# si220/Forest-SLAM

Measured on AMD Instinct MI355X. Metric: stereo frames/sec (extract+match+local-BA) at 600p, 1/8 MI355X; ATE RMSE, higher is better.
Workload: dtype mixed: u8/u16 integer (FAST, BRIEF, Hamming, SGM), f32 (ORB angle/Harris, back-projection), f64 (PnP, BA incl. its Schur GEMM on f64 MFMA); 1 GPU; stereo VO front end, configs[1]: 960x600, ORB nfeatures=1000, BF-Hamming xcheck (L+R), SGBM-3way 96 disp, back-projection, PnP-RANSAC, local BA K=10; width=960, height=600, nfeatures=1000, local_ba=window K=10 per frame, 10 LM iterations (fvo_ba_windows), parallelism=seq-per-gpu x1

## Files before the change

### forest-slam_amd/csrc/fvo_internal.h

```cpp
#pragma once

#include <hip/hip_runtime.h>

#include <cstdint>
#include <string>
#include <vector>

#include "../../include/fvo.h"

#define FVO_MAX_LEVELS 12

struct OrbGeom {
  int nlevels;
  int w[FVO_MAX_LEVELS], h[FVO_MAX_LEVELS];
  float scale[FVO_MAX_LEVELS];
  int64_t off[FVO_MAX_LEVELS + 1];
  int row0[FVO_MAX_LEVELS + 1];
  int nfeat[FVO_MAX_LEVELS];
  int64_t cand_off[FVO_MAX_LEVELS + 1];
  int64_t total_px;
  int total_rows;
  int64_t cand_total;
  bool angle_pass;
};
// ... 2 lines not shown
  int32_t* xofs;
  int32_t* xc1;
  int32_t* yofs;
  int32_t* yc1;
  int64_t xoff[FVO_MAX_LEVELS], yoff[FVO_MAX_LEVELS];
};

constexpr int kBaMaxWindow = 21;
constexpr int kEmMaxCap = 5040;
constexpr int kRansacMaxIters = 1000;

#define FVO_KERNELS(X)                                                                                    \
  X(KN_ORB_COPY, "orb_copy_level0") X(KN_ORB_RESIZE, "orb_resize") X(KN_ORB_FAST, "orb_fast_score")       \
  X(KN_ORB_NMS_COUNT, "orb_nms_count") X(KN_ORB_ROW_SCAN, "orb_row_scan") X(KN_ORB_COMPACT, "orb_nms_compact") \
  X(KN_ORB_SELECT1, "orb_select_fast") X(KN_ORB_HARRIS, "orb_harris") X(KN_ORB_SELECT2, "orb_select_harris") \
  X(KN_ORB_OFFSETS, "orb_offsets") X(KN_ORB_ANGLE, "orb_angle") X(KN_ORB_BLUR, "orb_blur")                \
  X(KN_ORB_BRIEF, "orb_brief") X(KN_BF_ARGMIN, "bf_argmin") X(KN_BF_FINISH, "bf_finish")                  \
  X(KN_SG_VERT, "sgbm_vert") X(KN_SG_ROWS, "sgbm_rows") X(KN_SG_MEDIAN, "sgbm_median")                    \
  X(KN_BACKPROJECT, "backproject") X(KN_PNP, "pnp_ransac") X(KN_BA_STEREO, "ba_stereo")                   \
  X(KN_BA_BUILD, "ba_build") X(KN_BA_SOLVE, "ba_solve") X(KN_GATHER, "gather_matches")                    \
  X(KN_ESSENTIAL, "essential_ransac") X(KN_RECOVER, "recover_pose") X(KN_INGEST, "ingest_undistort_gray") \
  X(KN_MOTION_BLUR, "motion_blur") X(KN_MAP_XFORM, "map_transform") X(KN_VOXEL, "voxel_down_sample")      \
  X(KN_BF_KNN, "bf_knn") X(KN_BF_RATIO, "bf_ratio") X(KN_SPK_LOCAL, "speckle_local")                      \
  X(KN_SPK_SEAMS, "speckle_seams") X(KN_SPK_SUM, "speckle_sum") X(KN_SPK_APPLY, "speckle_apply")
#define FVO_KERNEL_ID(id, name) id,
enum FvoKernel { FVO_KERNELS(FVO_KERNEL_ID) KN_COUNT };
#undef FVO_KERNEL_ID

struct TimingRec {
  int id;
  hipEvent_t a, b;
};

struct fvo_ctx {
  int device = 0;
  uint64_t tmask = 0;
  std::vector<TimingRec> trecs;
  std::vector<hipEvent_t> tpool;
  fvo_config cfg{};
  OrbGeom g{};
  std::string err;
  int kp_cap = 0;
  int64_t ws_bytes = 0;
  std::vector<void*> allocs;
  uint8_t* pyr = nullptr;
  uint8_t* blur = nullptr;
  int orb_last_batch = 0;
  uint8_t* score = nullptr;
  uint32_t* cand = nullptr;
  uint64_t* hel = nullptr;
  int32_t* ncand = nullptr;
  int32_t* nsel1 = nullptr;
  int32_t* nsel2 = nullptr;
  int32_t* koff = nullptr;
  int32_t* scratch = nullptr;
  int64_t scratch_per = 0;
  ResizeTab rt{};
  int32_t* umax = nullptr;
  uint32_t* bf_rowkey = nullptr;
  uint32_t* bf_colkey = nullptr;
  uint32_t* bf_knn = nullptr;
  uint16_t* sg_V = nullptr;
  uint16_t* sg_M = nullptr;
  uint32_t* sg_ckpt = nullptr;
  int16_t* sg_raw = nullptr;
  uint64_t* sg_hand = nullptr;
  uint32_t* sg_ctl = nullptr;
  struct {
    bool valid = false;
    const void* matches = nullptr;
    const void* nmatch = nullptr;
    const void* stereo = nullptr;
    int nframes = 0, first_end = 0, nwin = 0, first_valid = 0;
  } ba_births;
  double* pnp_hyp = nullptr;
  int32_t* pnp_sub = nullptr;
  int16_t* rs_table = nullptr;
  int32_t rs_table_iters = 0;
  double* pnp_models = nullptr;
  double* pnp_ws = nullptr;
  int32_t* pnp_good = nullptr;
  void* pnp_state = nullptr;
  float* pnp_pts = nullptr;
  int32_t* pnp_plan = nullptr;
  int32_t pnp_max_iters = 0;
  uint8_t* fast_rec = nullptr;
  void* ba_ws = nullptr;
  int64_t ba_win_bytes = 0;
  hipStream_t ba_s2 = nullptr;
  hipEvent_t ba_fork = nullptr, ba_join = nullptr;
  double* em_x = nullptr;
  double* em_models = nullptr;
  int32_t* em_good = nullptr;
  int8_t* em_nmod = nullptr;
  double* em_ws = nullptr;
  void* em_state = nullptr;
  int32_t em_max_iters = 0;
  int32_t rectify_budget = FVO_RECTIFY_LDS_BYTES;
};

int fvo_fail(fvo_ctx* ctx, const std::string& msg);
#define FVO_HIP(ctx, expr)                                                                 \
  do {                                                                                     \
    hipError_t e_ = (expr);                                                                \
    if (e_ != hipSuccess) return fvo_fail(ctx, std::string(#expr) + ": " + hipGetErrorString(e_)); \
  } while (0)
#define FVO_LAUNCH_CHECK(ctx) FVO_HIP(ctx, hipGetLastError())

hipEvent_t fvo_event(fvo_ctx* ctx);
#define FVO_TIMED(ctx, id, s, ...)                               \
  do {                                                           \
    const bool t_ = ((ctx)->tmask >> (id)) & 1ull;               \
    hipEvent_t a_ = nullptr, b_ = nullptr;                       \
    if (t_) {                                                    \
      a_ = fvo_event(ctx);                                       \
      (void)hipEventRecord(a_, s);                               \
    }                                                            \
    __VA_ARGS__;                                                 \
    if (t_) {                                                    \
      b_ = fvo_event(ctx);                                       \
      (void)hipEventRecord(b_, s);                               \
      (ctx)->trecs.push_back(TimingRec{(int)(id), a_, b_});      \
    }                                                            \
  } while (0)

int orb_init(fvo_ctx* ctx);
int orb_run(fvo_ctx* ctx, const uint8_t* images, int batch, int64_t image_stride, int pitch, float* kp, uint8_t* desc,
            int32_t* counts, int cap, hipStream_t s);
int bf_init(fvo_ctx* ctx);
int bf_run(fvo_ctx* ctx, const uint8_t* q, const int32_t* nq, const uint8_t* t, const int32_t* nt, int batch, int cap,
           int32_t* matches, int32_t* nmatch, hipStream_t s);
int bf_knn_run(fvo_ctx* ctx, const uint8_t* q, const int32_t* nq, const uint8_t* t, const int32_t* nt, int batch,
               int cap, int k, int32_t* knn, hipStream_t s);
int bf_ratio_run(fvo_ctx* ctx, const uint8_t* q, const int32_t* nq, const uint8_t* t, const int32_t* nt, int batch,
                 int cap, double ratio, int mutual, int32_t* matches, int32_t* nmatch, hipStream_t s);
int sgbm_init(fvo_ctx* ctx);
int sgbm_run(fvo_ctx* ctx, const uint8_t* L, const uint8_t* R, int batch, int64_t image_stride, int pitch,
             int16_t* disp, int32_t* status, hipStream_t s);
int pose_init(fvo_ctx* ctx);
int ransac_table_init(fvo_ctx* ctx);
int orb_blur_debug(fvo_ctx* ctx);
int orb_score_debug(fvo_ctx* ctx);
int orb_retain_best_run(fvo_ctx* ctx, const float* keys, int n, int keep, int32_t* idx_out, int32_t* n_out,
                         hipStream_t s);
int backproject_run(fvo_ctx* ctx, const int16_t* disp, const float* kp0, const float* kp1, const int32_t* matches,
                    const int32_t* nmatch, int batch, int cap, const double* K, double baseline, float* P3, float* p2,
                    int32_t* npts, hipStream_t s);
int pnp_run(fvo_ctx* ctx, const float* P3, const float* p2, const int32_t* npts, int batch, int cap, const double* K,
            const double* dist, float reproj, double conf, int iters, double* rvec, double* tvec, double* T,
            int32_t* status, uint8_t* inliers, hipStream_t s);

int ingest_run(fvo_ctx* ctx, const uint8_t* bgr, int batch, int64_t sstride, int spitch, const double* K,
               const double* dist, uint8_t* gray, int64_t dstride, int dpitch, hipStream_t s);
int motion_blur_run(fvo_ctx* ctx, const uint8_t* img, int batch, int64_t sstride, int spitch, int ksize,
                    const int32_t* centers, const int32_t* ncent, int cap, uint8_t* mask, uint8_t* out,
                    int64_t dstride, int dpitch, hipStream_t s);
int map_transform_run(fvo_ctx* ctx, const float* pts, int stride, const int32_t* npts, int batch, int64_t cap,
                      const double* T, int32_t* count, int64_t map_cap, double* out64, float* out32, hipStream_t s);
int chain_poses_run(fvo_ctx* ctx, const double* T, const int32_t* status, const int32_t* npts, int n_seq, int n,
                    double* cum, double* cum_out, int32_t* npts_out, hipStream_t s);
struct FvoRegions {
  fvo_region r[FVO_MAX_REGIONS];
};
int copy_regions_run(fvo_ctx* ctx, int count, const fvo_region* regions, hipStream_t s);
int count_guard_run(fvo_ctx* ctx, const int32_t* cnt, const int32_t* q_cnt, int n, int sets, int32_t* status,
                    int32_t code, int32_t* nkp_out, hipStream_t s);
int64_t voxel_workspace_bytes(int64_t n);
// ... 60 lines not shown
```

### forest-slam_amd/csrc/pose.hip

```cpp
#include <cfloat>
#include <cstdlib>
#include <type_traits>

#include "fvo_device.h"
#include "ransac.h"

namespace {

constexpr int kChunk = 64;

constexpr int kBackprojectThreads = 256;

__global__ __launch_bounds__(kBackprojectThreads) void k_backproject(
    const int16_t* __restrict__ disp, const float* __restrict__ kp0, const float* __restrict__ kp1,
    const int32_t* __restrict__ matches, const int32_t* __restrict__ nmatch, int W, int H, int cap, StereoCamF K,
    float* __restrict__ P3, float* __restrict__ p2, int32_t* __restrict__ npts) {
  const int b = blockIdx.x;
  int n = nmatch[b];
  n = n < 0 ? 0 : (n > cap ? cap : n);
  __shared__ int s_w[16];
  __shared__ int s_carry;
  if (threadIdx.x == 0) s_carry = 0;
  __syncthreads();
  for (int base = 0; base < n; base += kBackprojectThreads) {
// ... 685 lines not shown
    double sum2 = 0.0;
    #pragma unroll
    for (int i = 0; i < NP; ++i) {
      const double* pw = &pws[3 * i];
      double Xc = dot3(&R[0], pw) + t[0], Yc = dot3(&R[3], pw) + t[1];
      double iz = 1.0 / (dot3(&R[6], pw) + t[2]);
      double ue = uc + fu * Xc * iz, ve = vc + fv * Yc * iz;
      double u = us[2 * i], v = us[2 * i + 1];
      sum2 += sqrt((u - ue) * (u - ue) + (v - ve) * (v - ve));
    }
    return sum2 / NP;
  }
  __device__ static void qr_solve(double* A, double* b, double* X) {
    const int nr = 6, nc = 4;
    double A1[4], A2[4];
    #pragma unroll
    for (int k = 0; k < nc; ++k) {
      double eta = fabs(A[k * nc + k]);
      #pragma unroll
      for (int i = k + 1; i < nr; ++i) eta = fmax(eta, fabs(A[i * nc + k]));
      if (eta == 0) return;
      double sum2 = 0.0, inv = 1. / eta;
      #pragma unroll
      for (int i = k; i < nr; ++i) {
        A[i * nc + k] *= inv;
        sum2 += A[i * nc + k] * A[i * nc + k];
      }
      double sigma = sqrt(sum2);
      if (A[k * nc + k] < 0) sigma = -sigma;
      A[k * nc + k] += sigma;
      A1[k] = sigma * A[k * nc + k];
      A2[k] = -eta * sigma;
      #pragma unroll
      for (int j = k + 1; j < nc; ++j) {
        double sum = 0;
        #pragma unroll
        for (int i = k; i < nr; ++i) sum += A[i * nc + k] * A[i * nc + j];
        double tau = sum / A1[k];
        #pragma unroll
        for (int i = k; i < nr; ++i) A[i * nc + j] -= tau * A[i * nc + k];
      }
    }
    #pragma unroll
    for (int j = 0; j < nc; ++j) {
      double tau = 0;
      #pragma unroll
      for (int i = j; i < nr; ++i) tau += A[i * nc + j] * b[i];
      tau /= A1[j];
      #pragma unroll
      for (int i = j; i < nr; ++i) b[i] -= tau * A[i * nc + j];
    }
    X[nc - 1] = b[nc - 1] / A2[nc - 1];
    #pragma unroll
    for (int i = nc - 2; i >= 0; --i) {
      double sum = 0;
      #pragma unroll
      for (int j = i + 1; j < nc; ++j) sum += A[i * nc + j] * X[j];
      X[i] = (b[i] - sum) / A2[i];
    }
  }
  __device__ static void gauss_newton(const double* L, const double* rho, double* betas) {
#pragma nounroll
    for (int it = 0; it < 5; ++it) {
      double A[24], b[6], x[4] = {0, 0, 0, 0};
      int o = 0;
      asm volatile("" : "+v"(o));
      #pragma unroll
      for (int i = 0; i < 6; ++i) {
        const double* r = L + o + 10 * i;
        A[i * 4 + 0] = 2 * r[0] * betas[0] + r[1] * betas[1] + r[3] * betas[2] + r[6] * betas[3];
        A[i * 4 + 1] = r[1] * betas[0] + 2 * r[2] * betas[1] + r[4] * betas[2] + r[7] * betas[3];
        A[i * 4 + 2] = r[3] * betas[0] + r[4] * betas[1] + 2 * r[5] * betas[2] + r[8] * betas[3];
        A[i * 4 + 3] = r[6] * betas[0] + r[7] * betas[1] + r[8] * betas[2] + 2 * r[9] * betas[3];
        b[i] = rho[o + i] - (r[0] * betas[0] * betas[0] + r[1] * betas[0] * betas[1] + r[2] * betas[1] * betas[1] +
                         r[3] * betas[0] * betas[2] + r[4] * betas[1] * betas[2] + r[5] * betas[2] * betas[2] +
                         r[6] * betas[0] * betas[3] + r[7] * betas[1] * betas[3] + r[8] * betas[2] * betas[3] +
                         r[9] * betas[3] * betas[3]);
      }
      qr_solve(A, b, x);
      #pragma unroll
      for (int i = 0; i < 4; ++i) betas[i] += x[i];
    }
  }
  template <int S>
  __device__ void build_mtm(double* __restrict__ MtM) {
    choose_control_points();
    barycentric();
#pragma unroll
    for (int i = 0; i < 144; ++i) MtM[i * S] = 0.0;
#pragma unroll
    for (int i = 0; i < NP; ++i) {
      const double* as = &alphas[4 * i];
      double u = us[2 * i], v = us[2 * i + 1];
      double M1[12], M2[12];
#pragma unroll
      for (int j = 0; j < 4; ++j) {
        M1[3 * j] = as[j] * fu; M1[3 * j + 1] = 0.0; M1[3 * j + 2] = as[j] * (uc - u);
        M2[3 * j] = 0.0; M2[3 * j + 1] = as[j] * fv; M2[3 * j + 2] = as[j] * (vc - v);
      }
#pragma unroll
      for (int a = 0; a < 12; ++a)
#pragma unroll
        for (int bb = 0; bb < 12; ++bb) MtM[(a * 12 + bb) * S] += M1[a] * M1[bb];
#pragma unroll
      for (int a = 0; a < 12; ++a)
#pragma unroll
        for (int bb = 0; bb < 12; ++bb) MtM[(a * 12 + bb) * S] += M2[a] * M2[bb];
    }
  }
  __device__ void prep(const double (*nv)[12], double* L, double* rho) const {
    const double* vv[4] = {nv[3], nv[2], nv[1], nv[0]};
    constexpr int pa[6] = {0, 0, 0, 1, 1, 2}, pb[6] = {1, 2, 3, 2, 3, 3};
#pragma unroll
    for (int i = 0; i < 6; ++i) {
      double dv[4][3];
#pragma unroll
      for (int a = 0; a < 4; ++a)
#pragma unroll
        for (int k = 0; k < 3; ++k) dv[a][k] = vv[a][3 * pa[i] + k] - vv[a][3 * pb[i] + k];
      double* r = L + 10 * i;
      r[0] = dot3(dv[0], dv[0]);
      r[1] = 2.0f * dot3(dv[0], dv[1]);
      r[2] = dot3(dv[1], dv[1]);
      r[3] = 2.0f * dot3(dv[0], dv[2]);
      r[4] = 2.0f * dot3(dv[1], dv[2]);
      r[5] = dot3(dv[2], dv[2]);
      r[6] = 2.0f * dot3(dv[0], dv[3]);
      r[7] = 2.0f * dot3(dv[1], dv[3]);
      r[8] = 2.0f * dot3(dv[2], dv[3]);
      r[9] = dot3(dv[3], dv[3]);
    }
    rho[0] = dist2(cws[0], cws[1]); rho[1] = dist2(cws[0], cws[2]); rho[2] = dist2(cws[0], cws[3]);
    rho[3] = dist2(cws[1], cws[2]); rho[4] = dist2(cws[1], cws[3]); rho[5] = dist2(cws[2], cws[3]);
  }
  __device__ double approx(int N, const double* L, const double* rho, const double (*nv)[12], double* R, double* t) {
    double betas[4];
    if (N == 1) {
      double A[24], b4[4];
      constexpr int c[4] = {0, 1, 3, 6};
#pragma unroll
      for (int i = 0; i < 6; ++i)
#pragma unroll
        for (int j = 0; j < 4; ++j) A[i * 4 + j] = L[i * 10 + c[j]];
      dsolve<6, 4>(A, rho, b4);
      double s = b4[0] < 0 ? -1.0 : 1.0;
      betas[0] = sqrt(s * b4[0]);
      betas[1] = s * b4[1] / betas[0];
      betas[2] = s * b4[2] / betas[0];
      betas[3] = s * b4[3] / betas[0];
    } else if (N == 2) {
      double A[18], b3[3];
#pragma unroll
      for (int i = 0; i < 6; ++i)
#pragma unroll
        for (int j = 0; j < 3; ++j) A[i * 3 + j] = L[i * 10 + j];
      dsolve<6, 3>(A, rho, b3);
      if (b3[0] < 0) {
        betas[0] = sqrt(-b3[0]);
        betas[1] = (b3[2] < 0) ? sqrt(-b3[2]) : 0.0;
      } else {
        betas[0] = sqrt(b3[0]);
        betas[1] = (b3[2] > 0) ? sqrt(b3[2]) : 0.0;
      }
      if (b3[1] < 0) betas[0] = -betas[0];
      betas[2] = 0.0;
      betas[3] = 0.0;
    } else {
      double A[30], b5[5];
#pragma unroll
      for (int i = 0; i < 6; ++i)
#pragma unroll
        for (int j = 0; j < 5; ++j) A[i * 5 + j] = L[i * 10 + j];
      dsolve<6, 5>(A, rho, b5);
      if (b5[0] < 0) {
        betas[0] = sqrt(-b5[0]);
        betas[1] = (b5[2] < 0) ? sqrt(-b5[2]) : 0.0;
      } else {
        betas[0] = sqrt(b5[0]);
        betas[1] = (b5[2] > 0) ? sqrt(b5[2]) : 0.0;
      }
      if (b5[1] < 0) betas[0] = -betas[0];
      betas[2] = b5[3] / betas[0];
      betas[3] = 0.0;
    }
    gauss_newton(L, rho, betas);
    return compute_R_and_t(nv, betas, R, t);
  }
};

using fvo_rs::RNG;
using fvo_rs::update_num_iters;

// ... 215 lines not shown
      for (int i = 0; i < 9; ++i) Rt[i] = -Rt[i];
#pragma unroll
    for (int i = 0; i < 3; ++i) T[i] = -(Rt[i * 3] * Mc[0] + Rt[i * 3 + 1] * Mc[1] + Rt[i * 3 + 2] * Mc[2]);
    if (lane == 0) {
#pragma unroll
      for (int i = 0; i < 9; ++i) sh.rt[i] = Rt[i];
#pragma unroll
      for (int i = 0; i < 3; ++i) sh.t3[i] = T[i];
    }
    for (int i = lane; i < n; i += 64) {
      const int j = i;
      double s0 = P3[3 * j], s1 = P3[3 * j + 1], s2 = P3[3 * j + 2];
      double X = Rt[0] * s0 + Rt[1] * s1 + Rt[2] * s2 + T[0];
      double Y = Rt[3] * s0 + Rt[4] * s1 + Rt[5] * s2 + T[1];
      double u = mn[2 * i], v = mn[2 * i + 1];
      double r0[9] = {X, Y, 1, 0, 0, 0, -u * X, -u * Y, -u};
      double r1[9] = {0, 0, 0, X, Y, 1, -v * X, -v * Y, -v};
      int k = 0;
#pragma unroll
      for (int a = 0; a < 9; ++a)
#pragma unroll
        for (int b = a; b < 9; ++b) LLp[k++] += r0[a] * r0[b] + r1[a] * r1[b];
    }
  }
#pragma unroll
  for (int k = 0; k < 78; ++k) {
    const double t = wave_sum(LLp[k]);
    if (lane == 0) sh.llp[k] = t;
  }
  __syncthreads();
  if (!planar) dlt12_null(sh.llp, sh.dlt[1], sh.dlt[2], sh.rrt);
  if (lane == 0) dlt_pose(sh, planar);
  __syncthreads();
  double prev[6];
  double lambdaLg10 = -3, prevErrNorm = DBL_MAX;
  int iters = 0;
  for (;;) {
    double e0 = lm_eval(sh, K, P3, p2, n, true);
#pragma unroll
    for (int i = 0; i < 6; ++i) prev[i] = sh.param[i];
    if (lane == 0) {
#pragma unroll
      for (int i = 0; i < 6; ++i) sh.prev[i] = prev[i];
    }
    __syncthreads();
    if (lane == 0) lm_step(sh, lambdaLg10);
    __syncthreads();
    if (iters == 0) prevErrNorm = e0;
    double errNorm;
    for (;;) {
      errNorm = lm_eval(sh, K, P3, p2, n, false);
      if (errNorm > prevErrNorm && ++lambdaLg10 <= 16) {
        if (lane == 0) lm_step(sh, lambdaLg10);
        __syncthreads();
        continue;
      }
      break;
    }
    lambdaLg10 = fmax(lambdaLg10 - 1, -16.0);
    double dn = 0, pn = 0;
#pragma unroll
    for (int i = 0; i < 6; ++i) {
      dn += (sh.param[i] - prev[i]) * (sh.param[i] - prev[i]);
      pn += prev[i] * prev[i];
    }
    double rel = sqrt(dn) / (sqrt(pn) + DBL_EPSILON);
    if (++iters >= 20 || rel < FLT_EPSILON) break;
    prevErrNorm = errNorm;
  }
  if (lane == 0) sh.flag = 1;
  __syncthreads();
}

struct PnpState {
  int maxGood, niters, best_it, n;
};

__global__ void k_pnp_table(int cap, int maxIters, int16_t* __restrict__ table) {
  const int n = blockIdx.x * blockDim.x + threadIdx.x;
  if (n < 6 || n > cap) return;
  fvo_rs::draw_subsets(n, maxIters, table + (int64_t)n * maxIters * 5);
}

__global__ void k_pnp_subsets(const int32_t* __restrict__ npts, int batch, int cap, int maxIters,
                              PnpState* __restrict__ state) {
  const int b = blockIdx.x * blockDim.x + threadIdx.x;
  if (b >= batch) return;
  int n = npts[b];
  n = n < 0 ? 0 : (n > cap ? cap : n);
  PnpState st;
  st.maxGood = 0;
  st.niters = maxIters;
  st.best_it = -1;
  st.n = n;
  state[b] = st;
}

constexpr int PNP_WS = 256;
constexpr int PW_NV = 0, PW_CWS = 48, PW_AL = 60, PW_PWS = 80, PW_US = 95, PW_MTM = 112;

constexpr int PNP_FIRST = 128;
constexpr int PNP_CS = 64, PNP_CA = 8, PNP_CB = 16;

__global__ __launch_bounds__(64) void k_pnp_plan(int batch, int maxIters, const PnpState* __restrict__ state,
                                                 int32_t* __restrict__ plan) {
  const int lane = threadIdx.x;
  int carry[3] = {0, 0, 0};
  const int C[3] = {PNP_CS, PNP_CA, PNP_CB};
  for (int b0 = 0; b0 < batch; b0 += 64) {
    const int b = b0 + lane;
    int rem = 0;
    if (b < batch) {
      const PnpState st = state[b];
      if (st.n >= 6) rem = max(0, min(st.niters, maxIters) - PNP_FIRST);
    }
#pragma unroll
    for (int k = 0; k < 3; ++k) {
      int v = (rem + C[k] - 1) / C[k];
#pragma unroll
      for (int o = 1; o < 64; o <<= 1) {
        const int y = __shfl_up(v, o, 64);
        if (lane >= o) v += y;
      }
      const int incl = v, excl = incl - (rem + C[k] - 1) / C[k];
      if (b < batch) plan[k * (batch + 1) + b] = carry[k] + excl;
      carry[k] += __shfl(incl, 63, 64);
    }
  }
  if (lane < 3) plan[lane * (batch + 1) + batch] = carry[lane];
}

__device__ __forceinline__ void pnp_unit(const int32_t* __restrict__ pre, int batch, int u, int C, int& b, int& base) {
  int lo = 0, hi = batch - 1;
  while (lo < hi) {
    const int mid = (lo + hi + 1) >> 1;
    if (pre[mid] <= u) lo = mid; else hi = mid - 1;
  }
  b = lo;
  base = PNP_FIRST + (u - pre[lo]) * C;
}

template <int C, typename Body>
__device__ __forceinline__ void pnp_units(const int32_t* __restrict__ plan, int k, int batch, int maxIters,
                                          const PnpState* __restrict__ state, Body body) {
  const int32_t* pre = plan ? plan + k * (batch + 1) : nullptr;
  const int total = plan ? pre[batch] : (int)blockIdx.x + 1;
  for (int u = blockIdx.x; u < total; u += gridDim.x) {
    int b, base, lim;
    if (plan) {
      pnp_unit(pre, batch, u, C, b, base);
      lim = maxIters;
    } else {
      b = blockIdx.y;
      base = u * C;
      lim = PNP_FIRST;
    }
    const PnpState st = state[b];
    const int hi = min(min(st.niters, maxIters), lim);
    if (st.n < 6 || base >= hi) continue;
    body(b, base, hi, st.n);
  }
}

__global__ __launch_bounds__(64, 4) void k_pnp_setup(const float* __restrict__ P3all, const float* __restrict__ p2all,
                                                  int cap, Cam K, int maxIters, int batch,
                                                  const int32_t* __restrict__ plan,
                                                  const int16_t* __restrict__ table, int table_iters,
                                                  const PnpState* __restrict__ state, double* __restrict__ ws) {
  extern __shared__ __attribute__((aligned(16))) double smt[];
  double* mt = smt + threadIdx.x;
  pnp_units<PNP_CS>(plan, 0, batch, maxIters, state, [&](int b, int base, int hi, int n) {
    const int it = base + threadIdx.x;
    if (it >= hi) return;
    const float* __restrict__ P3 = P3all + (int64_t)b * cap * 3;
    const float* __restrict__ p2 = p2all + (int64_t)b * cap * 2;
    double* w = ws + ((int64_t)b * maxIters + it) * PNP_WS;
    const int16_t* sb = table + ((int64_t)n * table_iters + it) * 5;
    EPnPd<5> e;
    e.fu = K.fx; e.fv = K.fy; e.uc = K.cx; e.vc = K.cy;
#pragma unroll
    for (int i = 0; i < 5; ++i) {
      int j = sb[i];
#pragma unroll
      for (int c = 0; c < 3; ++c) e.pws[3 * i + c] = (double)P3[j * 3 + c];
      double xy[2];
      dundistort(K, (double)p2[j * 2], (double)p2[j * 2 + 1], xy);
      float fx = (float)xy[0], fy = (float)xy[1];
      e.us[2 * i] = fx * K.fx + K.cx;
      e.us[2 * i + 1] = fy * K.fy + K.cy;
    }
    e.build_mtm<64>(mt);
#pragma unroll 8
    for (int k = 0; k < 144; ++k) w[PW_MTM + k] = mt[k * 64];
#pragma unroll
    for (int r = 0; r < 4; ++r)
#pragma unroll
      for (int k = 0; k < 3; ++k) w[PW_CWS + r * 3 + k] = e.cws[r][k];
#pragma unroll
    for (int k = 0; k < 20; ++k) w[PW_AL + k] = e.alphas[k];
#pragma unroll
    for (int k = 0; k < 15; ++k) w[PW_PWS + k] = e.pws[k];
#pragma unroll
    for (int k = 0; k < 10; ++k) w[PW_US + k] = e.us[k];
  });
}

__global__ __launch_bounds__(64) void k_pnp_hyp_a(int maxIters, int batch, const int32_t* __restrict__ plan,
                                                  const PnpState* __restrict__ state, double* __restrict__ ws) {
  __shared__ double su[8][144];
  const int g = threadIdx.x >> 3, l = threadIdx.x & 7;
  double* u = su[g];
  pnp_units<PNP_CA>(plan, 1, batch, maxIters, state, [&](int b, int base, int hi, int) {
    const int it = base + g;
    if (it >= hi) return;
    double* w = ws + ((int64_t)b * maxIters + it) * PNP_WS;
    for (int k = l; k < 144; k += 8) u[k] = w[PW_MTM + k];
    __builtin_amdgcn_s_waitcnt(0);
    __builtin_amdgcn_wave_barrier();
    jacobi12_null4_group(u, l, w + PW_NV);
  });
}

__global__ __launch_bounds__(64, 3) void k_pnp_hyp_b(const float* __restrict__ P3all, const float* __restrict__ p2all,
                                                  int cap, Cam K, float thr2, int maxIters, int batch,
                                                  const int32_t* __restrict__ plan,
                                                  const PnpState* __restrict__ state, const double* __restrict__ ws,
                                                  double* __restrict__ model, int32_t* __restrict__ good) {
  __shared__ double sL[16][66];
  const int g = threadIdx.x >> 2, l = threadIdx.x & 3;
  double* L = sL[g];
  pnp_units<PNP_CB>(plan, 2, batch, maxIters, state, [&](int b, int base, int hi, int n) {
    const int it = base + g;
    if (it >= hi) return;
    const float* __restrict__ P3 = P3all + (int64_t)b * cap * 3;
    const float* __restrict__ p2 = p2all + (int64_t)b * cap * 2;
    const double* w = ws + ((int64_t)b * maxIters + it) * PNP_WS;
    EPnPd<5, true> e;
    e.fu = K.fx; e.fv = K.fy; e.uc = K.cx; e.vc = K.cy;
    e.pws = w + PW_PWS;
    e.us = w + PW_US;
    e.alphas = w + PW_AL;
    e.cws = reinterpret_cast<const double (*)[3]>(w + PW_CWS);
    const double (*nv)[12] = reinterpret_cast<const double (*)[12]>(w + PW_NV);
    if (l == 0) e.prep(nv, L, L + 60);
    __builtin_amdgcn_s_waitcnt(0);
    __builtin_amdgcn_wave_barrier();
    double R[9], t[3];
    const double err = e.approx(l < 3 ? l + 1 : 3, L, L + 60, nv, R, t);
    const int gb = threadIdx.x & ~3;
    const double e1 = __shfl(err, gb + 1, 64), e2 = __shfl(err, gb + 2, 64);
    int sel = 0;
    double best = __shfl(err, gb, 64);
    if (e1 < best) { best = e1; sel = 1; }
    if (e2 < best) sel = 2;
#pragma unroll
    for (int k = 0; k < 9; ++k) R[k] = __shfl(R[k], gb + sel, 64);
#pragma unroll
    for (int k = 0; k < 3; ++k) t[k] = __shfl(t[k], gb + sel, 64);
    double r[3], dR[27];
    rod_R2r(R, r);
    if (l == 0) {
      double* mo = model + ((int64_t)b * maxIters + it) * 6;
      for (int i = 0; i < 3; ++i) { mo[i] = r[i]; mo[3 + i] = t[i]; }
    }
    rod_r2R(r, R, dR);
    int gcount = 0;
#pragma nounroll
    for (int i = l; i < n; i += 4) {
      double M[3] = {(double)P3[3 * i], (double)P3[3 * i + 1], (double)P3[3 * i + 2]}, uv[2];
      dproject(K, R, dR, t, M, uv, nullptr);
      float du = p2[2 * i] - (float)uv[0], dv = p2[2 * i + 1] - (float)uv[1];
      gcount += (du * du + dv * dv) <= thr2;
    }
    gcount += __shfl_xor(gcount, 1, 4);
    gcount += __shfl_xor(gcount, 2, 4);
    if (l == 0) good[(int64_t)b * maxIters + it] = gcount;
  });
}

__global__ __launch_bounds__(64) void k_pnp_replay(int maxIters, int it_lo, int it_hi, double conf,
                                                   const int32_t* __restrict__ good, PnpState* __restrict__ state) {
  const int b = blockIdx.x, lane = threadIdx.x;
  PnpState st = state[b];
  if (st.n < 6) return;
  for (int base = it_lo; base < it_hi && base < st.niters; base += 64) {
    const int it = base + lane;
    const int g = (it < it_hi && it < st.niters) ? good[(int64_t)b * maxIters + it] : 0;
    for (int j = 0; j < 64; ++j) {
      if (base + j >= it_hi || base + j >= st.niters) break;
      const int gj = __builtin_amdgcn_readlane(g, j);
      if (gj > max(st.maxGood, 4)) {
        st.best_it = base + j;
        st.maxGood = gj;
        st.niters = update_num_iters(conf, (double)(st.n - gj) / st.n, 5, st.niters);
      }
    }
  }
  if (lane == 0) state[b] = st;
}

__global__ __launch_bounds__(64, 2) void k_pnp_refine(const float* __restrict__ P3all, const float* __restrict__ p2all,
                                                   int cap, Cam K, float thr2, int maxIters,
                                                   const PnpState* __restrict__ state,
                                                   const double* __restrict__ model, double* __restrict__ rvec,
                                                   double* __restrict__ tvec, double* __restrict__ T,
                                                   int32_t* __restrict__ status, uint8_t* __restrict__ inliers,
                                                   int32_t* __restrict__ inl_idx, double* __restrict__ mn_buf,
                                                   float* __restrict__ pts) {
  __shared__ PnpShared sh;
  __shared__ float s_pts[5 * kRefineLds];
  const int b = blockIdx.x, lane = threadIdx.x;
  const PnpState st = state[b];
  const int n = st.n;
  const float* P3 = P3all + (int64_t)b * cap * 3;
  const float* p2 = p2all + (int64_t)b * cap * 2;
  double* Tout = T + (int64_t)b * 16;
  if (n < 6 || st.maxGood <= 0) {
    if (lane < 16) Tout[lane] = (lane % 5 == 0) ? 1.0 : 0.0;
    if (lane < 3) { rvec[b * 3 + lane] = 0; tvec[b * 3 + lane] = 0; }
    if (inliers)
      for (int i = lane; i < cap; i += 64) inliers[(int64_t)b * cap + i] = 0;
    if (lane == 0) status[b] = n < 6 ? -1 : 0;
    return;
  }
  const double* mo = model + ((int64_t)b * maxIters + st.best_it) * 6;
  if (lane < 6) sh.best[lane] = mo[lane];
  __syncthreads();
  int* inl = inl_idx + (int64_t)b * cap;
  {
    double r[3] = {sh.best[0], sh.best[1], sh.best[2]}, t[3] = {sh.best[3], sh.best[4], sh.best[5]};
    double R[9], dR[27];
    rod_r2R(r, R, dR);
    int carry = 0;
    for (int base = 0; base < n; base += 64) {
      int i = base + lane;
      bool f = false;
      if (i < n) {
        double M[3] = {(double)P3[3 * i], (double)P3[3 * i + 1], (double)P3[3 * i + 2]}, uv[2];
        dproject(K, R, dR, t, M, uv, nullptr);
        float du = p2[2 * i] - (float)uv[0], dv = p2[2 * i + 1] - (float)uv[1];
        f = du * du + dv * dv <= thr2;
        if (inliers) inliers[(int64_t)b * cap + i] = (uint8_t)f;
      }
      unsigned long long m = __ballot(f);
      if (f) {
        const int k = carry + __popcll(m & ((1ull << lane) - 1ull));
        inl[k] = i;
        if (k < kRefineLds) {
          s_pts[3 * k] = P3[3 * i];
          s_pts[3 * k + 1] = P3[3 * i + 1];
          s_pts[3 * k + 2] = P3[3 * i + 2];
          s_pts[3 * kRefineLds + 2 * k] = p2[2 * i];
          s_pts[3 * kRefineLds + 2 * k + 1] = p2[2 * i + 1];
        }
      }
      carry += __popcll(m);
    }
    if (inliers)
      for (int i = n + lane; i < cap; i += 64) inliers[(int64_t)b * cap + i] = 0;
    if (lane == 0) sh.ninl = carry;
  }
  __syncthreads();
  const int ninl = sh.ninl;
  const float* Pc = s_pts;
  const float* Qc = s_pts + 3 * kRefineLds;
  if (ninl > kRefineLds) {
    float* gP = pts + (int64_t)b * cap * 5;
    float* gQ = gP + 3 * cap;
    for (int k = lane; k < ninl; k += 64) {
      const int i = inl[k];
      gP[3 * k] = P3[3 * i];
      gP[3 * k + 1] = P3[3 * i + 1];
      gP[3 * k + 2] = P3[3 * i + 2];
      gQ[2 * k] = p2[2 * i];
      gQ[2 * k + 1] = p2[2 * i + 1];
    }
    __syncthreads();
    Pc = gP;
    Qc = gQ;
  }
  lm_refine(sh, K, Pc, Qc, ninl, mn_buf + (int64_t)b * cap * 2);
  double out[6];
  for (int i = 0; i < 6; ++i) out[i] = sh.flag ? sh.param[i] : sh.best[i];
  if (lane == 0) {
    double R[9];
    rod_r2R(out, R, nullptr);
    for (int i = 0; i < 3; ++i) {
      rvec[b * 3 + i] = out[i];
      tvec[b * 3 + i] = out[3 + i];
      Tout[i * 4 + 0] = R[i * 3];
      Tout[i * 4 + 1] = R[i * 3 + 1];
      Tout[i * 4 + 2] = R[i * 3 + 2];
      Tout[i * 4 + 3] = out[3 + i];
    }
    Tout[12] = 0; Tout[13] = 0; Tout[14] = 0; Tout[15] = 1;
    status[b] = 1;
  }
}

}

int pose_init(fvo_ctx* ctx) {
  ctx->pnp_max_iters = kRansacMaxIters;
  const int64_t B = ctx->cfg.max_batch, n = B * ctx->kp_cap, it = B * ctx->pnp_max_iters;
  int rc;
  if ((rc = fvo_alloc(ctx, &ctx->pnp_sub, n)) || (rc = fvo_alloc(ctx, &ctx->pnp_hyp, 2 * n)) ||
      (rc = ransac_table_init(ctx)) || (rc = fvo_alloc(ctx, &ctx->pnp_models, it * 6)) ||
      (rc = fvo_alloc(ctx, &ctx->pnp_ws, it * PNP_WS)) ||
      (rc = hipFuncSetAttribute((const void*)k_pnp_setup, hipFuncAttributeMaxDynamicSharedMemorySize,
                                144 * 64 * (int)sizeof(double)) == hipSuccess ? 0 : fvo_fail(ctx, "pnp: LDS attribute")) ||
      (rc = fvo_alloc(ctx, &ctx->pnp_good, it)) || (rc = fvo_alloc(ctx, (PnpState**)&ctx->pnp_state, B)) ||
      (rc = fvo_alloc(ctx, &ctx->pnp_plan, 3 * (B + 1))) || (rc = fvo_alloc(ctx, &ctx->pnp_pts, 5 * n)))
    return rc;
  return 0;
}

int ransac_table_init(fvo_ctx* ctx) {
  if (ctx->rs_table) return 0;
  ctx->rs_table_iters = kRansacMaxIters;
  int rc;
  if ((rc = fvo_alloc(ctx, &ctx->rs_table, (int64_t)(ctx->kp_cap + 1) * ctx->rs_table_iters * 5))) return rc;
  hipLaunchKernelGGL(k_pnp_table, dim3((ctx->kp_cap + 1 + 63) / 64), dim3(64), 0, 0, ctx->kp_cap,
                     ctx->rs_table_iters, ctx->rs_table);
  FVO_LAUNCH_CHECK(ctx);
  FVO_HIP(ctx, hipDeviceSynchronize());
  return 0;
}

int backproject_run(fvo_ctx* ctx, const int16_t* disp, const float* kp0, const float* kp1, const int32_t* matches,
                    const int32_t* nmatch, int batch, int cap, const double* K, double baseline, float* P3, float* p2,
                    int32_t* npts, hipStream_t s) {
  FVO_TIMED(ctx, KN_BACKPROJECT, s,
            hipLaunchKernelGGL(k_backproject, dim3(batch), dim3(kBackprojectThreads), 0, s, disp, kp0, kp1, matches,
                               nmatch, ctx->cfg.width, ctx->cfg.height, cap, stereo_cam(K, baseline), P3, p2, npts));
  FVO_LAUNCH_CHECK(ctx);
  return 0;
}

int pnp_run(fvo_ctx* ctx, const float* P3, const float* p2, const int32_t* npts, int batch, int cap, const double* K,
            const double* dist, float reproj, double conf, int iters, double* rvec, double* tvec, double* T,
            int32_t* status, uint8_t* inliers, hipStream_t s) {
  Cam c{K[0], K[4], K[2], K[5], {dist[0], dist[1], dist[2], dist[3], dist[4]}};
  const float thr2 = (float)((double)reproj * reproj);
  const int maxIters = iters;
  PnpState* st = (PnpState*)ctx->pnp_state;
  const int first = std::min(maxIters, PNP_FIRST);
  auto hyp = [&](const int32_t* plan, dim3 gs, dim3 ga, dim3 gb, int lo, int hi) {
    hipLaunchKernelGGL(k_pnp_setup, gs, dim3(64), 144 * 64 * sizeof(double), s, P3, p2, cap, c, maxIters, batch, plan,
                       ctx->rs_table, ctx->rs_table_iters, st, ctx->pnp_ws);
    hipLaunchKernelGGL(k_pnp_hyp_a, ga, dim3(64), 0, s, maxIters, batch, plan, st, ctx->pnp_ws);
    hipLaunchKernelGGL(k_pnp_hyp_b, gb, dim3(64), 0, s, P3, p2, cap, c, thr2, maxIters, batch, plan, st, ctx->pnp_ws,
                       ctx->pnp_models, ctx->pnp_good);
    hipLaunchKernelGGL(k_pnp_replay, dim3(batch), dim3(64), 0, s, maxIters, lo, hi, conf, ctx->pnp_good, st);
  };
  FVO_TIMED(ctx, KN_PNP, s, {
    hipLaunchKernelGGL(k_pnp_subsets, dim3((batch + 63) / 64), dim3(64), 0, s, npts, batch, cap, maxIters, st);
    hyp(nullptr, dim3((first + PNP_CS - 1) / PNP_CS, batch), dim3((first + PNP_CA - 1) / PNP_CA, batch),
        dim3((first + PNP_CB - 1) / PNP_CB, batch), 0, first);
    if (maxIters > first) {
      hipLaunchKernelGGL(k_pnp_plan, dim3(1), dim3(64), 0, s, batch, maxIters, st, ctx->pnp_plan);
      const int gs = batch * ((PNP_FIRST + PNP_CS - 1) / PNP_CS), ga = batch * ((PNP_FIRST + PNP_CA - 1) / PNP_CA),
                gb = batch * ((PNP_FIRST + PNP_CB - 1) / PNP_CB);
      hyp(ctx->pnp_plan, dim3(gs), dim3(ga), dim3(gb), first, maxIters);
    }
    hipLaunchKernelGGL(k_pnp_refine, dim3(batch), dim3(64), 0, s, P3, p2, cap, c, thr2, maxIters, st,
                       ctx->pnp_models, rvec, tvec, T, status, inliers, ctx->pnp_sub, ctx->pnp_hyp, ctx->pnp_pts);
  });
  FVO_LAUNCH_CHECK(ctx);
  return 0;
}
```

Before: 6000 frames/s.

## Fuse PnP setup into null-space kernel and fold plan, init and replay into neighbours

Measured after the change: 6033 frames/s, median of 6. No clear change (+0.6%).

```diff
diff --git a/forest-slam_amd/csrc/fvo_internal.h b/forest-slam_amd/csrc/fvo_internal.h
--- a/forest-slam_amd/csrc/fvo_internal.h
+++ b/forest-slam_amd/csrc/fvo_internal.h
@@ -108,7 +108,6 @@
   int32_t* pnp_good = nullptr;
   void* pnp_state = nullptr;
   float* pnp_pts = nullptr;
-  int32_t* pnp_plan = nullptr;
   int32_t pnp_max_iters = 0;
   uint8_t* fast_rec = nullptr;
   void* ba_ws = nullptr;
diff --git a/forest-slam_amd/csrc/pose.hip b/forest-slam_amd/csrc/pose.hip
--- a/forest-slam_amd/csrc/pose.hip
+++ b/forest-slam_amd/csrc/pose.hip
@@ -791,32 +791,6 @@
       for (int i = 0; i < 4; ++i) betas[i] += x[i];
     }
   }
-  template <int S>
-  __device__ void build_mtm(double* __restrict__ MtM) {
-    choose_control_points();
-    barycentric();
-#pragma unroll
-    for (int i = 0; i < 144; ++i) MtM[i * S] = 0.0;
-#pragma unroll
-    for (int i = 0; i < NP; ++i) {
-      const double* as = &alphas[4 * i];
-      double u = us[2 * i], v = us[2 * i + 1];
-      double M1[12], M2[12];
-#pragma unroll
-      for (int j = 0; j < 4; ++j) {
-        M1[3 * j] = as[j] * fu; M1[3 * j + 1] = 0.0; M1[3 * j + 2] = as[j] * (uc - u);
-        M2[3 * j] = 0.0; M2[3 * j + 1] = as[j] * fv; M2[3 * j + 2] = as[j] * (vc - v);
-      }
-#pragma unroll
-      for (int a = 0; a < 12; ++a)
-#pragma unroll
-        for (int bb = 0; bb < 12; ++bb) MtM[(a * 12 + bb) * S] += M1[a] * M1[bb];
-#pragma unroll
-      for (int a = 0; a < 12; ++a)
-#pragma unroll
-        for (int bb = 0; bb < 12; ++bb) MtM[(a * 12 + bb) * S] += M2[a] * M2[bb];
-    }
-  }
   __device__ void prep(const double (*nv)[12], double* L, double* rho) const {
     const double* vv[4] = {nv[3], nv[2], nv[1], nv[0]};
     constexpr int pa[6] = {0, 0, 0, 1, 1, 2}, pb[6] = {1, 2, 3, 2, 3, 3};
@@ -1198,139 +1172,144 @@
   fvo_rs::draw_subsets(n, maxIters, table + (int64_t)n * maxIters * 5);
 }
 
-__global__ void k_pnp_subsets(const int32_t* __restrict__ npts, int batch, int cap, int maxIters,
-                              PnpState* __restrict__ state) {
-  const int b = blockIdx.x * blockDim.x + threadIdx.x;
-  if (b >= batch) return;
-  int n = npts[b];
-  n = n < 0 ? 0 : (n > cap ? cap : n);
-  PnpState st;
-  st.maxGood = 0;
-  st.niters = maxIters;
-  st.best_it = -1;
-  st.n = n;
-  state[b] = st;
-}
-
-constexpr int PNP_WS = 256;
-constexpr int PW_NV = 0, PW_CWS = 48, PW_AL = 60, PW_PWS = 80, PW_US = 95, PW_MTM = 112;
+constexpr int PNP_WS = 112;
+constexpr int PW_NV = 0, PW_CWS = 48, PW_AL = 60, PW_PWS = 80, PW_US = 95;
 
 constexpr int PNP_FIRST = 128;
-constexpr int PNP_CS = 64, PNP_CA = 8, PNP_CB = 16;
-
-__global__ __launch_bounds__(64) void k_pnp_plan(int batch, int maxIters, const PnpState* __restrict__ state,
-                                                 int32_t* __restrict__ plan) {
+constexpr int PNP_CA = 8, PNP_CB = 16;
+
+__device__ __forceinline__ int pnp_clamp_n(int n, int cap) { return n < 0 ? 0 : (n > cap ? cap : n); }
+
+template <int C, typename Body>
+__device__ __forceinline__ void pnp_units(int batch, int cap, int maxIters,
+                                          const int32_t* __restrict__ npts, const PnpState* __restrict__ state,
+                                          Body body) {
+  __shared__ int pre[4][64];
   const int lane = threadIdx.x;
-  int carry[3] = {0, 0, 0};
-  const int C[3] = {PNP_CS, PNP_CA, PNP_CB};
-  for (int b0 = 0; b0 < batch; b0 += 64) {
-    const int b = b0 + lane;
-    int rem = 0;
-    if (b < batch) {
-      const PnpState st = state[b];
-      if (st.n >= 6) rem = max(0, min(st.niters, maxIters) - PNP_FIRST);
-    }
-#pragma unroll
-    for (int k = 0; k < 3; ++k) {
-      int v = (rem + C[k] - 1) / C[k];
+  const bool round2 = npts == nullptr;
+  int u = blockIdx.x, tot = 0;
+  for (int b0 = 0; b0 < (round2 ? batch : 1); b0 += 64) {
+    if (!round2) {
+      tot = u + 1;
+    } else {
+      const int bl = b0 + lane;
+      int n = 0, nit = 0, v = 0;
+      if (bl < batch) {
+        const PnpState st = state[bl];
+        n = st.n;
+        nit = min(st.niters, maxIters);
+        if (n >= 6) v = (max(0, nit - PNP_FIRST) + C - 1) / C;
+      }
+      int incl = v;
 #pragma unroll
       for (int o = 1; o < 64; o <<= 1) {
-        const int y = __shfl_up(v, o, 64);
-        if (lane >= o) v += y;
-      }
-      const int incl = v, excl = incl - (rem + C[k] - 1) / C[k];
-      if (b < batch) plan[k * (batch + 1) + b] = carry[k] + excl;
-      carry[k] += __shfl(incl, 63, 64);
-    }
-  }
-  if (lane < 3) plan[lane * (batch + 1) + batch] = carry[lane];
-}
-
-__device__ __forceinline__ void pnp_unit(const int32_t* __restrict__ pre, int batch, int u, int C, int& b, int& base) {
-  int lo = 0, hi = batch - 1;
-  while (lo < hi) {
-    const int mid = (lo + hi + 1) >> 1;
-    if (pre[mid] <= u) lo = mid; else hi = mid - 1;
-  }
-  b = lo;
-  base = PNP_FIRST + (u - pre[lo]) * C;
-}
-
-template <int C, typename Body>
-__device__ __forceinline__ void pnp_units(const int32_t* __restrict__ plan, int k, int batch, int maxIters,
-                                          const PnpState* __restrict__ state, Body body) {
-  const int32_t* pre = plan ? plan + k * (batch + 1) : nullptr;
-  const int total = plan ? pre[batch] : (int)blockIdx.x + 1;
-  for (int u = blockIdx.x; u < total; u += gridDim.x) {
-    int b, base, lim;
-    if (plan) {
-      pnp_unit(pre, batch, u, C, b, base);
-      lim = maxIters;
-    } else {
-      b = blockIdx.y;
-      base = u * C;
-      lim = PNP_FIRST;
-    }
-    const PnpState st = state[b];
-    const int hi = min(min(st.niters, maxIters), lim);
-    if (st.n < 6 || base >= hi) continue;
-    body(b, base, hi, st.n);
-  }
-}
-
-__global__ __launch_bounds__(64, 4) void k_pnp_setup(const float* __restrict__ P3all, const float* __restrict__ p2all,
-                                                  int cap, Cam K, int maxIters, int batch,
-                                                  const int32_t* __restrict__ plan,
-                                                  const int16_t* __restrict__ table, int table_iters,
-                                                  const PnpState* __restrict__ state, double* __restrict__ ws) {
-  extern __shared__ __attribute__((aligned(16))) double smt[];
-  double* mt = smt + threadIdx.x;
-  pnp_units<PNP_CS>(plan, 0, batch, maxIters, state, [&](int b, int base, int hi, int n) {
-    const int it = base + threadIdx.x;
+        const int y = __shfl_up(incl, o, 64);
+        if (lane >= o) incl += y;
+      }
+      incl += tot;
+      __builtin_amdgcn_wave_barrier();
+      pre[0][lane] = incl - v;
+      pre[1][lane] = incl;
+      pre[2][lane] = nit;
+      pre[3][lane] = n;
+      __builtin_amdgcn_s_waitcnt(0);
+      __builtin_amdgcn_wave_barrier();
+      tot = __shfl(incl, 63, 64);
+    }
+    while (u < tot) {
+      int b, base, hi, nn;
+      if (round2) {
+        const int src = __ffsll((unsigned long long)__ballot(pre[0][lane] <= u && u < pre[1][lane])) - 1;
+        b = b0 + src;
+        base = PNP_FIRST + (u - pre[0][src]) * C;
+        hi = pre[2][src];
+        nn = pre[3][src];
+      } else {
+        b = blockIdx.y;
+        base = u * C;
+        hi = min(maxIters, PNP_FIRST);
+        nn = pnp_clamp_n(npts[b], cap);
+      }
+      b = __builtin_amdgcn_readfirstlane(b);
+      base = __builtin_amdgcn_readfirstlane(base);
+      hi = __builtin_amdgcn_readfirstlane(hi);
+      nn = __builtin_amdgcn_readfirstlane(nn);
+      if (nn >= 6 && base < hi) body(b, base, hi, nn);
+      u += gridDim.x;
+    }
+  }
+}
+
+__global__ __launch_bounds__(64, 4) void k_pnp_null(const float* __restrict__ P3all, const float* __restrict__ p2all,
+                                                 const int32_t* __restrict__ npts, int cap, Cam K, int maxIters,
+                                                 int batch, const int16_t* __restrict__ table,
+                                                 int table_iters, const PnpState* __restrict__ state,
+                                                 double* __restrict__ ws) {
+  __shared__ double su[8][144];
+  __shared__ double sa[8][32];
+  const int g = threadIdx.x >> 3, l = threadIdx.x & 7;
+  double* u = su[g];
+  double* al = sa[g];
+  pnp_units<PNP_CA>(batch, cap, maxIters, npts, state, [&](int b, int base, int hi, int n) {
+    const int it = base + g;
     if (it >= hi) return;
     const float* __restrict__ P3 = P3all + (int64_t)b * cap * 3;
     const float* __restrict__ p2 = p2all + (int64_t)b * cap * 2;
     double* w = ws + ((int64_t)b * maxIters + it) * PNP_WS;
     const int16_t* sb = table + ((int64_t)n * table_iters + it) * 5;
-    EPnPd<5> e;
-    e.fu = K.fx; e.fv = K.fy; e.uc = K.cx; e.vc = K.cy;
-#pragma unroll
-    for (int i = 0; i < 5; ++i) {
-      int j = sb[i];
-#pragma unroll
-      for (int c = 0; c < 3; ++c) e.pws[3 * i + c] = (double)P3[j * 3 + c];
-      double xy[2];
-      dundistort(K, (double)p2[j * 2], (double)p2[j * 2 + 1], xy);
-      float fx = (float)xy[0], fy = (float)xy[1];
-      e.us[2 * i] = fx * K.fx + K.cx;
-      e.us[2 * i + 1] = fy * K.fy + K.cy;
-    }
-    e.build_mtm<64>(mt);
-#pragma unroll 8
-    for (int k = 0; k < 144; ++k) w[PW_MTM + k] = mt[k * 64];
-#pragma unroll
-    for (int r = 0; r < 4; ++r)
-#pragma unroll
-      for (int k = 0; k < 3; ++k) w[PW_CWS + r * 3 + k] = e.cws[r][k];
-#pragma unroll
-    for (int k = 0; k < 20; ++k) w[PW_AL + k] = e.alphas[k];
-#pragma unroll
-    for (int k = 0; k < 15; ++k) w[PW_PWS + k] = e.pws[k];
-#pragma unroll
-    for (int k = 0; k < 10; ++k) w[PW_US + k] = e.us[k];
-  });
-}
-
-__global__ __launch_bounds__(64) void k_pnp_hyp_a(int maxIters, int batch, const int32_t* __restrict__ plan,
-                                                  const PnpState* __restrict__ state, double* __restrict__ ws) {
-  __shared__ double su[8][144];
-  const int g = threadIdx.x >> 3, l = threadIdx.x & 7;
-  double* u = su[g];
-  pnp_units<PNP_CA>(plan, 1, batch, maxIters, state, [&](int b, int base, int hi, int) {
-    const int it = base + g;
-    if (it >= hi) return;
-    double* w = ws + ((int64_t)b * maxIters + it) * PNP_WS;
-    for (int k = l; k < 144; k += 8) u[k] = w[PW_MTM + k];
+    {
+      EPnPd<5> e;
+      e.fu = K.fx; e.fv = K.fy; e.uc = K.cx; e.vc = K.cy;
+#pragma unroll
+      for (int i = 0; i < 5; ++i) {
+        int j = sb[i];
+#pragma unroll
+        for (int c = 0; c < 3; ++c) e.pws[3 * i + c] = (double)P3[j * 3 + c];
+        double xy[2];
+        dundistort(K, (double)p2[j * 2], (double)p2[j * 2 + 1], xy);
+        float fx = (float)xy[0], fy = (float)xy[1];
+        e.us[2 * i] = fx * K.fx + K.cx;
+        e.us[2 * i + 1] = fy * K.fy + K.cy;
+      }
+      e.choose_control_points();
+      e.barycentric();
+      if (l == 0) {
+#pragma unroll
+        for (int k = 0; k < 20; ++k) al[k] = e.alphas[k];
+#pragma unroll
+        for (int k = 0; k < 10; ++k) al[20 + k] = e.us[k];
+#pragma unroll
+        for (int r = 0; r < 4; ++r)
+#pragma unroll
+          for (int k = 0; k < 3; ++k) w[PW_CWS + r * 3 + k] = e.cws[r][k];
+#pragma unroll
+        for (int k = 0; k < 20; ++k) w[PW_AL + k] = e.alphas[k];
+#pragma unroll
+        for (int k = 0; k < 15; ++k) w[PW_PWS + k] = e.pws[k];
+#pragma unroll
+        for (int k = 0; k < 10; ++k) w[PW_US + k] = e.us[k];
+      }
+    }
+    __builtin_amdgcn_s_waitcnt(0);
+    __builtin_amdgcn_wave_barrier();
+#pragma nounroll
+    for (int k = l; k < 144; k += 8) {
+      const int a = k / 12, bb = k - a * 12;
+      const int ja = a / 3, ca = a - ja * 3, jb = bb / 3, cb = bb - jb * 3;
+      double m = 0.0;
+#pragma unroll
+      for (int i = 0; i < 5; ++i) {
+        const double asa = al[4 * i + ja], asb = al[4 * i + jb];
+        const double pu = al[20 + 2 * i], pv = al[20 + 2 * i + 1];
+        const double m1a = ca == 0 ? asa * K.fx : (ca == 1 ? 0.0 : asa * (K.cx - pu));
+        const double m1b = cb == 0 ? asb * K.fx : (cb == 1 ? 0.0 : asb * (K.cx - pu));
+        const double m2a = ca == 0 ? 0.0 : (ca == 1 ? asa * K.fy : asa * (K.cy - pv));
+        const double m2b = cb == 0 ? 0.0 : (cb == 1 ? asb * K.fy : asb * (K.cy - pv));
+        m += m1a * m1b;
+        m += m2a * m2b;
+      }
+      u[k] = m;
+    }
     __builtin_amdgcn_s_waitcnt(0);
     __builtin_amdgcn_wave_barrier();
     jacobi12_null4_group(u, l, w + PW_NV);
@@ -1338,14 +1317,14 @@
 }
 
 __global__ __launch_bounds__(64, 3) void k_pnp_hyp_b(const float* __restrict__ P3all, const float* __restrict__ p2all,
-                                                  int cap, Cam K, float thr2, int maxIters, int batch,
-                                                  const int32_t* __restrict__ plan,
+                                                  const int32_t* __restrict__ npts, int cap, Cam K, float thr2,
+                                                  int maxIters, int batch,
                                                   const PnpState* __restrict__ state, const double* __restrict__ ws,
                                                   double* __restrict__ model, int32_t* __restrict__ good) {
   __shared__ double sL[16][66];
   const int g = threadIdx.x >> 2, l = threadIdx.x & 3;
   double* L = sL[g];
-  pnp_units<PNP_CB>(plan, 2, batch, maxIters, state, [&](int b, int base, int hi, int n) {
+  pnp_units<PNP_CB>(batch, cap, maxIters, npts, state, [&](int b, int base, int hi, int n) {
     const int it = base + g;
     if (it >= hi) return;
     const float* __restrict__ P3 = P3all + (int64_t)b * cap * 3;
@@ -1394,11 +1373,8 @@
   });
 }
 
-__global__ __launch_bounds__(64) void k_pnp_replay(int maxIters, int it_lo, int it_hi, double conf,
-                                                   const int32_t* __restrict__ good, PnpState* __restrict__ state) {
-  const int b = blockIdx.x, lane = threadIdx.x;
-  PnpState st = state[b];
-  if (st.n < 6) return;
+__device__ __forceinline__ void pnp_replay(PnpState& st, int b, int lane, int maxIters, int it_lo, int it_hi,
+                                           double conf, const int32_t* __restrict__ good) {
   for (int base = it_lo; base < it_hi && base < st.niters; base += 64) {
     const int it = base + lane;
     const int g = (it < it_hi && it < st.niters) ? good[(int64_t)b * maxIters + it] : 0;
@@ -1412,12 +1388,25 @@
       }
     }
   }
+}
+
+__global__ __launch_bounds__(64) void k_pnp_replay(const int32_t* __restrict__ npts, int cap, int maxIters, int it_hi,
+                                                   double conf, const int32_t* __restrict__ good,
+                                                   PnpState* __restrict__ state) {
+  const int b = blockIdx.x, lane = threadIdx.x;
+  PnpState st;
+  st.maxGood = 0;
+  st.niters = maxIters;
+  st.best_it = -1;
+  st.n = pnp_clamp_n(npts[b], cap);
+  if (st.n >= 6) pnp_replay(st, b, lane, maxIters, 0, it_hi, conf, good);
   if (lane == 0) state[b] = st;
 }
 
 __global__ __launch_bounds__(64, 2) void k_pnp_refine(const float* __restrict__ P3all, const float* __restrict__ p2all,
-                                                   int cap, Cam K, float thr2, int maxIters,
-                                                   const PnpState* __restrict__ state,
+                                                   int cap, Cam K, float thr2, int maxIters, double conf,
+                                                   PnpState* __restrict__ state,
+                                                   const int32_t* __restrict__ good,
                                                    const double* __restrict__ model, double* __restrict__ rvec,
                                                    double* __restrict__ tvec, double* __restrict__ T,
                                                    int32_t* __restrict__ status, uint8_t* __restrict__ inliers,
@@ -1426,8 +1415,12 @@
   __shared__ PnpShared sh;
   __shared__ float s_pts[5 * kRefineLds];
   const int b = blockIdx.x, lane = threadIdx.x;
-  const PnpState st = state[b];
+  PnpState st = state[b];
   const int n = st.n;
+  if (n >= 6 && maxIters > PNP_FIRST) {
+    pnp_replay(st, b, lane, maxIters, PNP_FIRST, maxIters, conf, good);
+    if (lane == 0) state[b] = st;
+  }
   const float* P3 = P3all + (int64_t)b * cap * 3;
   const float* p2 = p2all + (int64_t)b * cap * 2;
   double* Tout = T + (int64_t)b * 16;
@@ -1523,10 +1516,8 @@
   if ((rc = fvo_alloc(ctx, &ctx->pnp_sub, n)) || (rc = fvo_alloc(ctx, &ctx->pnp_hyp, 2 * n)) ||
       (rc = ransac_table_init(ctx)) || (rc = fvo_alloc(ctx, &ctx->pnp_models, it * 6)) ||
       (rc = fvo_alloc(ctx, &ctx->pnp_ws, it * PNP_WS)) ||
-      (rc = hipFuncSetAttribute((const void*)k_pnp_setup, hipFuncAttributeMaxDynamicSharedMemorySize,
-                                144 * 64 * (int)sizeof(double)) == hipSuccess ? 0 : fvo_fail(ctx, "pnp: LDS attribute")) ||
       (rc = fvo_alloc(ctx, &ctx->pnp_good, it)) || (rc = fvo_alloc(ctx, (PnpState**)&ctx->pnp_state, B)) ||
-      (rc = fvo_alloc(ctx, &ctx->pnp_plan, 3 * (B + 1))) || (rc = fvo_alloc(ctx, &ctx->pnp_pts, 5 * n)))
+      (rc = fvo_alloc(ctx, &ctx->pnp_pts, 5 * n)))
     return rc;
   return 0;
 }
@@ -1561,26 +1552,19 @@
   const int maxIters = iters;
   PnpState* st = (PnpState*)ctx->pnp_state;
   const int first = std::min(maxIters, PNP_FIRST);
-  auto hyp = [&](const int32_t* plan, dim3 gs, dim3 ga, dim3 gb, int lo, int hi) {
-    hipLaunchKernelGGL(k_pnp_setup, gs, dim3(64), 144 * 64 * sizeof(double), s, P3, p2, cap, c, maxIters, batch, plan,
-                       ctx->rs_table, ctx->rs_table_iters, st, ctx->pnp_ws);
-    hipLaunchKernelGGL(k_pnp_hyp_a, ga, dim3(64), 0, s, maxIters, batch, plan, st, ctx->pnp_ws);
-    hipLaunchKernelGGL(k_pnp_hyp_b, gb, dim3(64), 0, s, P3, p2, cap, c, thr2, maxIters, batch, plan, st, ctx->pnp_ws,
-                       ctx->pnp_models, ctx->pnp_good);
-    hipLaunchKernelGGL(k_pnp_replay, dim3(batch), dim3(64), 0, s, maxIters, lo, hi, conf, ctx->pnp_good, st);
+  auto hyp = [&](const int32_t* npts, dim3 ga, dim3 gb) {
+    hipLaunchKernelGGL(k_pnp_null, ga, dim3(64), 0, s, P3, p2, npts, cap, c, maxIters, batch, ctx->rs_table,
+                       ctx->rs_table_iters, st, ctx->pnp_ws);
+    hipLaunchKernelGGL(k_pnp_hyp_b, gb, dim3(64), 0, s, P3, p2, npts, cap, c, thr2, maxIters, batch, st,
+                       ctx->pnp_ws, ctx->pnp_models, ctx->pnp_good);
   };
   FVO_TIMED(ctx, KN_PNP, s, {
-    hipLaunchKernelGGL(k_pnp_subsets, dim3((batch + 63) / 64), dim3(64), 0, s, npts, batch, cap, maxIters, st);
-    hyp(nullptr, dim3((first + PNP_CS - 1) / PNP_CS, batch), dim3((first + PNP_CA - 1) / PNP_CA, batch),
-        dim3((first + PNP_CB - 1) / PNP_CB, batch), 0, first);
-    if (maxIters > first) {
-      hipLaunchKernelGGL(k_pnp_plan, dim3(1), dim3(64), 0, s, batch, maxIters, st, ctx->pnp_plan);
-      const int gs = batch * ((PNP_FIRST + PNP_CS - 1) / PNP_CS), ga = batch * ((PNP_FIRST + PNP_CA - 1) / PNP_CA),
-                gb = batch * ((PNP_FIRST + PNP_CB - 1) / PNP_CB);
-      hyp(ctx->pnp_plan, dim3(gs), dim3(ga), dim3(gb), first, maxIters);
-    }
-    hipLaunchKernelGGL(k_pnp_refine, dim3(batch), dim3(64), 0, s, P3, p2, cap, c, thr2, maxIters, st,
-                       ctx->pnp_models, rvec, tvec, T, status, inliers, ctx->pnp_sub, ctx->pnp_hyp, ctx->pnp_pts);
+    hyp(npts, dim3((first + PNP_CA - 1) / PNP_CA, batch), dim3((first + PNP_CB - 1) / PNP_CB, batch));
+    hipLaunchKernelGGL(k_pnp_replay, dim3(batch), dim3(64), 0, s, npts, cap, maxIters, first, conf, ctx->pnp_good, st);
+    if (maxIters > first)
+      hyp(nullptr, dim3(batch * ((PNP_FIRST + PNP_CA - 1) / PNP_CA)), dim3(batch * ((PNP_FIRST + PNP_CB - 1) / PNP_CB)));
+    hipLaunchKernelGGL(k_pnp_refine, dim3(batch), dim3(64), 0, s, P3, p2, cap, c, thr2, maxIters, conf, st,
+                       ctx->pnp_good, ctx->pnp_models, rvec, tvec, T, status, inliers, ctx->pnp_sub, ctx->pnp_hyp, ctx->pnp_pts);
   });
   FVO_LAUNCH_CHECK(ctx);
   return 0;
diff --git a/profiles/pnp_chain/compare_dumps.py b/profiles/pnp_chain/compare_dumps.py
--- /dev/null
+++ b/profiles/pnp_chain/compare_dumps.py
@@ -0,0 +1,17 @@
+import os
+import sys
+
+import numpy as np
+
+a, b = sys.argv[1:3]
+names = sorted(f for f in os.listdir(a) if f.endswith(".npy"))
+assert names and names == sorted(f for f in os.listdir(b) if f.endswith(".npy")), (names, os.listdir(b))
+bad = []
+for f in names:
+    x, y = np.load(os.path.join(a, f)), np.load(os.path.join(b, f))
+    same = x.shape == y.shape and x.dtype == y.dtype and np.array_equal(x.view(np.uint8), y.view(np.uint8))
+    print(f"{f:32s} {str(x.dtype):8s} {str(x.shape):20s} {'equal' if same else 'DIFFERENT'}")
+    if not same:
+        bad.append(f)
+print(f"{len(names)} arrays, {len(bad)} different")
+sys.exit(1 if bad else 0)
```
